# jkulhanek/tetra-nerf

Measured on NVIDIA H100. Metric: rays/sec (4096-ray batch, 300k-tet mesh), higher is better.
Workload: dtype f32 (trace/interp/compositing) + f16w2 tensor-core MLP (fp16 activations x fp16 hi/lo weights, f32 accumulate; per-sample density/colour within 1e-4 of the fp32 oracle, tests/test_gpu_render.py)

## Files before the change

tetra-nerf_b200/csrc/tn_mlp.cuh:

```cuda
#pragma once
#include "tn_common.cuh"
#include "tn_tc.cuh"

namespace tn {

#ifndef TN_MLP_WGS
#define TN_MLP_WGS 3
#endif
constexpr uint32_t MLP_WGS = TN_MLP_WGS;
constexpr uint32_t MLP_THREADS = 128 * MLP_WGS;
constexpr uint32_t MLP_TILE = 64;
constexpr uint32_t MLP_W_BYTES = 32768 + 3 * 65536;
constexpr uint32_t MLP_W_COARSE = 32768 + 2 * 65536;
__host__ __device__ constexpr uint32_t mlp_off_head(bool fine) { return fine ? MLP_W_BYTES : MLP_W_COARSE; }
__host__ __device__ constexpr uint32_t mlp_off_bars(bool fine) { return mlp_off_head(fine) + 520 * 4; }
__host__ __device__ constexpr uint32_t mlp_smem_bytes(bool fine) { return mlp_off_bars(fine) + 8 + 8 * MLP_WGS; }
static_assert(mlp_smem_bytes(true) <= 232448, "k_mlp shared memory exceeds 227 KB");
__host__ __device__ constexpr uint32_t mlp_off_layer(int l) { return l == 0 ? 0u : 32768u + 65536u * (uint32_t)(l - 1); }

struct MlpParams {
    const uint32_t *n_active;
    uint32_t S;
    const uint4 *vi;
    const float *bary;
    const float *fshadow;
    const uint8_t *wimg;
    const float *bias;
    const float *head;
    const float *dirbias;
    float *out;
    uint32_t *tile_ctr;
    const uint32_t *rowmap;
    const uint32_t *n_rows;
};

constexpr uint32_t MLP_NO_TILE = 0xFFFFFFFFu;

__device__ __forceinline__ float softplus_f(float x) { return x > 20.0f ? x : log1pf(expf(x)); }
__device__ __forceinline__ float sigmoid_f(float x) { return 1.0f / (1.0f + expf(-x)); }

__device__ __forceinline__ float4 ldg_stream(const float4 *p) {
    float4 v;
    asm volatile("ld.global.nc.L1::no_allocate.v4.f32 {%0, %1, %2, %3}, [%4];" : "=f"(v.x), "=f"(v.y), "=f"(v.z), "=f"(v.w) : "l"(p));
    return v;
}
__device__ __forceinline__ float4 ldg_l1(const float4 *p) {
    float4 v;
    asm volatile("ld.global.nc.v4.f32 {%0, %1, %2, %3}, [%4];" : "=f"(v.x), "=f"(v.y), "=f"(v.z), "=f"(v.w) : "l"(p));
    return v;
}

template <bool ALLOC_L1>
__device__ __forceinline__ void load_field_quads(const float *__restrict__ row, uint32_t t, float4 (&q)[4]) {
#pragma unroll
    for (int kk = 0; kk < 4; ++kk) {
        const float4 *p = reinterpret_cast<const float4 *>(row + field_pos(16u * kk + 2u * t));
        q[kk] = ALLOC_L1 ? ldg_l1(p) : ldg_stream(p);
    }
}
__device__ __forceinline__ float2 field_pair(const float4 (&q)[4], int c) {
    const float4 v = q[c >> 1];
    return (c & 1) ? make_float2(v.z, v.w) : make_float2(v.x, v.y);
}

__device__ __forceinline__ void wg_sync(uint32_t wg) { asm volatile("bar.sync %0, 128;" ::"r"(1u + wg) : "memory"); }

template <int PREC>
__device__ __forceinline__ void to_operand(float e0, float e1, uint32_t &hi, uint32_t &lo) {
    if (PREC == 2) hi = tc::pack2_f16(e0, e1);
    else tc::split_pack2(e0, e1, hi, lo);
}

struct GatherRows {
    uint4 v[2];
    float b[2][3];
};
__device__ __forceinline__ GatherRows load_gather_rows(const uint4 *__restrict__ vi, const float *__restrict__ bary, uint64_t row0, uint64_t total_rows) {
    GatherRows r;
#pragma unroll
    for (int rr = 0; rr < 2; ++rr) {
        const uint64_t row = row0 + 8u * rr;
        r.v[rr] = make_uint4(TN_EMPTY, TN_EMPTY, TN_EMPTY, TN_EMPTY);
        r.b[rr][0] = r.b[rr][1] = r.b[rr][2] = 0.f;
        if (row < total_rows) {
            r.v[rr] = __ldg(vi + row);
            r.b[rr][0] = __ldg(bary + 3 * row); r.b[rr][1] = __ldg(bary + 3 * row + 1); r.b[rr][2] = __ldg(bary + 3 * row + 2);
        }
    }
    return r;
}
__device__ __forceinline__ GatherRows load_gather_rows_mapped(const uint4 *__restrict__ vi, const float *__restrict__ bary, const uint32_t *__restrict__ rowmap,
                                                          uint64_t row0, uint64_t total_rows) {
    GatherRows r;
#pragma unroll
    for (int rr = 0; rr < 2; ++rr) {
        const uint64_t row = row0 + 8u * rr;
        r.v[rr] = make_uint4(TN_EMPTY, TN_EMPTY, TN_EMPTY, TN_EMPTY);
        r.b[rr][0] = r.b[rr][1] = r.b[rr][2] = 0.f;
        if (row < total_rows) {
            const size_t s = __ldg(rowmap + row);
            r.v[rr] = __ldg(vi + s);
            r.b[rr][0] = __ldg(bary + 3 * s); r.b[rr][1] = __ldg(bary + 3 * s + 1); r.b[rr][2] = __ldg(bary + 3 * s + 2);
        }
    }
    return r;
}
__device__ __forceinline__ void prefetch_l1(const void *p) { asm volatile("prefetch.global.L1 [%0];" ::"l"(p)); }
__device__ __forceinline__ void prefetch_gather_rows(const uint4 *vi, const float *bary, uint64_t row0, uint64_t total_rows) {
#pragma unroll
    for (int rr = 0; rr < 2; ++rr) {
        const uint64_t row = row0 + 8u * rr;
        if (row < total_rows) {
            prefetch_l1(vi + row);
            prefetch_l1(bary + 3 * row);
        }
    }
}

template <int PREC, bool ALLOC_L1 = false>
__device__ __forceinline__ void gather_rows(const GatherRows &r, const float *__restrict__ fshadow, uint32_t t, uint32_t (&xh)[16], uint32_t (&xl)[16]) {
    float4 a[2][4][4];
#pragma unroll
    for (int rr = 0; rr < 2; ++rr) {
        const uint4 v = r.v[rr].x != TN_EMPTY ? r.v[rr] : make_uint4(0u, 0u, 0u, 0u);
        const uint32_t vs[4] = {v.x, v.y, v.z, v.w};
#pragma unroll
        for (int k = 0; k < 4; ++k) load_field_quads<ALLOC_L1>(fshadow + (size_t)vs[k] * 64, t, a[rr][k]);
    }
#pragma unroll
    for (int rr = 0; rr < 2; ++rr) {
        const bool m = r.v[rr].x != TN_EMPTY;
        const float b0 = r.b[rr][0], b1 = r.b[rr][1], b2 = r.b[rr][2];
        const float w0 = __fsub_rn(1.0f, __fadd_rn(__fadd_rn(b0, b1), b2));
#pragma unroll
        for (int c = 0; c < 8; ++c) {
            const float2 a0 = field_pair(a[rr][0], c), a1 = field_pair(a[rr][1], c), a2 = field_pair(a[rr][2], c), a3 = field_pair(a[rr][3], c);
            float2 o;
            o.x = __fmaf_rn(b0, a1.x, 0.f); o.y = __fmaf_rn(b0, a1.y, 0.f);
            o.x = __fmaf_rn(b1, a2.x, o.x); o.y = __fmaf_rn(b1, a2.y, o.y);
            o.x = __fmaf_rn(b2, a3.x, o.x); o.y = __fmaf_rn(b2, a3.y, o.y);
            o.x = __fmaf_rn(w0, a0.x, o.x); o.y = __fmaf_rn(w0, a0.y, o.y);
            if (!m) o = make_float2(0.f, 0.f);
            const int i = 4 * (c >> 1) + 2 * (c & 1) + rr;
            to_operand<PREC>(o.x, o.y, xh[i], xl[i]);
        }
    }
}

template <int PREC, int KSTEPS>
__device__ __forceinline__ void layer_mma(float (&d)[64], const uint32_t (&ah)[4 * KSTEPS], const uint32_t (&al)[4 * KSTEPS], uint32_t w) {
    using namespace tc;
    wgmma_fence();
#pragma unroll
    for (int kk = 0; kk < KSTEPS; ++kk) {
        const uint32_t wb = w + (uint32_t)(kk >> 2) * 32768u + (uint32_t)(kk & 3) * 32u;
        const uint32_t a[4] = {ah[4 * kk], ah[4 * kk + 1], ah[4 * kk + 2], ah[4 * kk + 3]};
        if (PREC == 2) {
            wgmma_rs_f16_n128<0>(d, a, make_desc(wb), kk > 0 ? 1u : 0u);
            wgmma_rs_f16_n128<0>(d, a, make_desc(wb + 16384u), 1u);
        } else {
            const uint32_t b[4] = {al[4 * kk], al[4 * kk + 1], al[4 * kk + 2], al[4 * kk + 3]};
            wgmma_rs_bf16_n128<0>(d, a, make_desc(wb), kk > 0 ? 1u : 0u);
            wgmma_rs_bf16_n128<0>(d, b, make_desc(wb), 1u);
            wgmma_rs_bf16_n128<0>(d, a, make_desc(wb + 16384u), 1u);
        }
    }
    wgmma_commit();
    wgmma_wait0();
    reg_fence(d);
}

template <bool FINE, int PREC, bool MAP = false>
__global__ void __launch_bounds__(MLP_THREADS, 1) k_mlp(const MlpParams p) {
    using namespace tc;
    extern __shared__ __align__(1024) uint8_t tn_mlp_smem[];
    uint8_t *smem = tn_mlp_smem;
    const float *head_s = reinterpret_cast<const float *>(smem + mlp_off_head(FINE));
    uint64_t *w_bar = reinterpret_cast<uint64_t *>(smem + mlp_off_bars(FINE));
    volatile uint32_t *slots = reinterpret_cast<volatile uint32_t *>(smem + mlp_off_bars(FINE) + 8);

    constexpr int L = FINE ? 4 : 3;
    constexpr uint32_t WBYTES = FINE ? MLP_W_BYTES : MLP_W_COARSE;
    const uint32_t wg = threadIdx.x >> 7, tid = threadIdx.x & 127u;
    const uint32_t warp = tid >> 5, lane = threadIdx.x & 31u, g = lane >> 2, t = lane & 3u;
    const uint32_t n_active = *p.n_active;
    const uint64_t total_rows = MAP ? (uint64_t)*p.n_rows : (uint64_t)n_active * p.S;
    const uint32_t ntiles = (uint32_t)((total_rows + MLP_TILE - 1) / MLP_TILE);
    if (blockIdx.x * MLP_WGS >= ntiles) return;
    auto sample_row = [&](uint64_t row) -> uint64_t { return MAP ? (uint64_t)__ldg(p.rowmap + row) : row; };

    if (threadIdx.x == 0) {
        mbar_init(w_bar, 1);
        fence_barrier_init();
    }
    for (uint32_t i = threadIdx.x; i < 516; i += MLP_THREADS) const_cast<float *>(head_s)[i] = p.head[i];
    auto draw = [&]() {
        const uint32_t nx = gridDim.x * MLP_WGS + atomicAdd(p.tile_ctr, 1u);
        return nx < ntiles ? nx : MLP_NO_TILE;
    };
    if (tid == 0) {
        const uint32_t first = blockIdx.x * MLP_WGS + wg;
        slots[2 * wg] = first < ntiles ? first : MLP_NO_TILE;
        slots[2 * wg + 1] = draw();
    }
    __syncthreads();
    if (threadIdx.x == 0) {
        mbar_arrive_expect_tx(w_bar, WBYTES);
        for (uint32_t off = 0; off < WBYTES; off += 16384) tma_bulk_g2s(smem + off, p.wimg + off, 16384, w_bar);
    }
    const uint32_t wsm = smem_u32(smem);
    const float *wd = head_s, *wc = head_s + 128;
    bool weights_ready = false;
    const uint32_t lrow = warp * 16u + g;
    uint32_t tile = slots[2 * wg];

#pragma unroll 1
    for (uint32_t n = 0;; ++n) {
        wg_sync(wg);
        if (tile == MLP_NO_TILE) break;
        const uint32_t next = slots[2 * wg + ((n + 1u) & 1u)];
        if (tid == 0) slots[2 * wg + (n & 1u)] = draw();
        const uint64_t row0 = (uint64_t)tile * MLP_TILE + lrow, row1 = row0 + 8u;
        const float *db0 = nullptr, *db1 = nullptr;

        uint32_t ah[32], al[32];
        {
            uint32_t xh[16], xl[16];
            if constexpr (MAP) gather_rows<PREC, true>(load_gather_rows_mapped(p.vi, p.bary, p.rowmap, row0, total_rows), p.fshadow, t, xh, xl);
            else gather_rows<PREC, true>(load_gather_rows(p.vi, p.bary, row0, total_rows), p.fshadow, t, xh, xl);
            if constexpr (MAP) { if (next != MLP_NO_TILE && lrow == warp * 16u) prefetch_l1(p.rowmap + (uint64_t)next * MLP_TILE + lrow); }
            else if (next != MLP_NO_TILE) prefetch_gather_rows(p.vi, p.bary, (uint64_t)next * MLP_TILE + lrow, total_rows);
            if (FINE) {
                db0 = p.dirbias + (size_t)((uint32_t)sample_row(min(row0, total_rows - 1)) / p.S) * 128;
                db1 = p.dirbias + (size_t)((uint32_t)sample_row(min(row1, total_rows - 1)) / p.S) * 128;
                prefetch_l1(db0 + 32 * t);
                prefetch_l1(db1 + 32 * t);
            }
            if (!weights_ready) { mbar_wait(w_bar, 0); weights_ready = true; }
            float d[64];
            layer_mma<PREC, 4>(d, xh, xl, wsm + mlp_off_layer(0));
#pragma unroll
            for (int j = 0; j < 16; ++j) {
                const float2 b = __ldg(reinterpret_cast<const float2 *>(p.bias + 8 * j + 2 * t));
                const int i = 4 * (j >> 1) + 2 * (j & 1);
                to_operand<PREC>(fmaxf(d[4 * j] + b.x, 0.f), fmaxf(d[4 * j + 1] + b.y, 0.f), ah[i], al[i]);
                to_operand<PREC>(fmaxf(d[4 * j + 2] + b.x, 0.f), fmaxf(d[4 * j + 3] + b.y, 0.f), ah[i + 1], al[i + 1]);
            }
        }
        float dens0 = 0.f, dens1 = 0.f;
#pragma unroll
        for (int l = 1; l < 3; ++l) {
            float d[64];
            layer_mma<PREC, 8>(d, ah, al, wsm + mlp_off_layer(l));
            const float *bias = p.bias + 128 * l;
#pragma unroll
            for (int j = 0; j < 16; ++j) {
                const int c = 8 * j + 2 * (int)t;
                const float2 b = __ldg(reinterpret_cast<const float2 *>(bias + c));
                const float x0 = fmaxf(d[4 * j] + b.x, 0.f), x1 = fmaxf(d[4 * j + 1] + b.y, 0.f);
                const float y0 = fmaxf(d[4 * j + 2] + b.x, 0.f), y1 = fmaxf(d[4 * j + 3] + b.y, 0.f);
                if (l == 2) {
                    dens0 = fmaf(x0, wd[c], dens0); dens0 = fmaf(x1, wd[c + 1], dens0);
                    dens1 = fmaf(y0, wd[c], dens1); dens1 = fmaf(y1, wd[c + 1], dens1);
                }
                if (l < L - 1) {
                    const int i = 4 * (j >> 1) + 2 * (j & 1);
                    to_operand<PREC>(x0, x1, ah[i], al[i]);
                    to_operand<PREC>(y0, y1, ah[i + 1], al[i + 1]);
                }
            }
        }
        float col0[3] = {0.f, 0.f, 0.f}, col1[3] = {0.f, 0.f, 0.f};
        if (FINE) {
            float d[64];
            layer_mma<PREC, 8>(d, ah, al, wsm + mlp_off_layer(3));
#pragma unroll
            for (int j = 0; j < 16; ++j) {
                const int c = 8 * j + 2 * (int)t;
                const float2 b0 = __ldg(reinterpret_cast<const float2 *>(db0 + c)), b1 = __ldg(reinterpret_cast<const float2 *>(db1 + c));
                const float x0 = fmaxf(d[4 * j] + b0.x, 0.f), x1 = fmaxf(d[4 * j + 1] + b0.y, 0.f);
                const float y0 = fmaxf(d[4 * j + 2] + b1.x, 0.f), y1 = fmaxf(d[4 * j + 3] + b1.y, 0.f);
#pragma unroll
                for (int ch = 0; ch < 3; ++ch) {
                    const float *w = wc + 128 * ch;
                    col0[ch] = fmaf(x1, w[c + 1], fmaf(x0, w[c], col0[ch]));
                    col1[ch] = fmaf(y1, w[c + 1], fmaf(y0, w[c], col1[ch]));
                }
            }
        }
#pragma unroll
        for (int s = 1; s <= 2; s <<= 1) {
            dens0 += __shfl_xor_sync(0xffffffffu, dens0, s);
            dens1 += __shfl_xor_sync(0xffffffffu, dens1, s);
            if (FINE) {
#pragma unroll
                for (int ch = 0; ch < 3; ++ch) {
                    col0[ch] += __shfl_xor_sync(0xffffffffu, col0[ch], s);
                    col1[ch] += __shfl_xor_sync(0xffffffffu, col1[ch], s);
                }
            }
        }
        if (t < 2) {
            const uint64_t row = t == 0 ? row0 : row1;
            const float dn = t == 0 ? dens0 : dens1;
            if (row < total_rows) {
                const uint64_t orow = sample_row(row);
                const float sigma = softplus_f(dn + head_s[512]);
                if (FINE) {
                    const float c0 = t == 0 ? col0[0] : col1[0], c1 = t == 0 ? col0[1] : col1[1], c2 = t == 0 ? col0[2] : col1[2];
                    reinterpret_cast<float4 *>(p.out)[orow] =
                        make_float4(sigma, sigmoid_f(c0 + head_s[513]), sigmoid_f(c1 + head_s[514]), sigmoid_f(c2 + head_s[515]));
                } else {
                    p.out[orow] = sigma;
                }
            }
        }
        tile = next;
    }
    if (!weights_ready) mbar_wait(w_bar, 0);
}

template <bool FINE, int PREC, bool MAP = false>
inline int launch_mlp(const MlpParams &p, uint32_t grid, cudaStream_t s) {
    auto k = k_mlp<FINE, PREC, MAP>;
    TN_CUDA(cudaFuncSetAttribute(k, cudaFuncAttributeMaxDynamicSharedMemorySize, (int)mlp_smem_bytes(FINE)));
    k<<<grid, MLP_THREADS, mlp_smem_bytes(FINE), s>>>(p);
    return TN_OK;
}

}
```

tetra-nerf_b200/csrc/tn_tc.cuh:

```cuda
#pragma once
#include <cuda_bf16.h>
#include <cuda_runtime.h>
#include <stdint.h>

namespace tn {
namespace tc {

__device__ __forceinline__ uint32_t smem_u32(const void *p) { return (uint32_t)__cvta_generic_to_shared(p); }

__device__ __forceinline__ void mbar_init(uint64_t *bar, uint32_t count) {
    asm volatile("mbarrier.init.shared::cta.b64 [%0], %1;" ::"r"(smem_u32(bar)), "r"(count));
}
__device__ __forceinline__ void fence_barrier_init() { asm volatile("fence.mbarrier_init.release.cluster;" ::: "memory"); }
__device__ __forceinline__ void mbar_arrive(uint64_t *bar) {
    asm volatile("mbarrier.arrive.shared::cta.b64 _, [%0];" ::"r"(smem_u32(bar)) : "memory");
}
__device__ __forceinline__ void mbar_arrive_expect_tx(uint64_t *bar, uint32_t bytes) {
    asm volatile("mbarrier.arrive.expect_tx.shared::cta.b64 _, [%0], %1;" ::"r"(smem_u32(bar)), "r"(bytes) : "memory");
}
__device__ __forceinline__ bool mbar_test(uint64_t *bar, uint32_t parity) {
    uint32_t ok;
    asm volatile(
        "{\n\t.reg .pred p;\n\t"
        "mbarrier.try_wait.parity.shared::cta.b64 p, [%1], %2;\n\t"
        "selp.u32 %0, 1, 0, p;\n\t}"
        : "=r"(ok)
        : "r"(smem_u32(bar)), "r"(parity)
        : "memory");
    return ok != 0;
}
__device__ __forceinline__ void mbar_wait(uint64_t *bar, uint32_t parity) {
    while (!mbar_test(bar, parity)) {}
}
__device__ __forceinline__ void mbar_wait_backoff(uint64_t *bar, uint32_t parity, uint32_t ns) {
    while (!mbar_test(bar, parity)) __nanosleep(ns);
}

__device__ __forceinline__ bool mbar_test_a(uint32_t bar, uint32_t parity) {
    uint32_t ok;
    asm volatile(
        "{\n\t.reg .pred p;\n\t"
        "mbarrier.try_wait.parity.shared::cta.b64 p, [%1], %2;\n\t"
        "selp.u32 %0, 1, 0, p;\n\t}"
        : "=r"(ok)
        : "r"(bar), "r"(parity)
        : "memory");
    return ok != 0;
}
__device__ __forceinline__ void mbar_wait_a(uint32_t bar, uint32_t parity) {
    while (!mbar_test_a(bar, parity)) {}
}
__device__ __forceinline__ void mbar_wait_backoff_a(uint32_t bar, uint32_t parity, uint32_t ns) {
    while (!mbar_test_a(bar, parity)) __nanosleep(ns);
}

__device__ __forceinline__ void tma_bulk_g2s(void *dst_smem, const void *src_gmem, uint32_t bytes, uint64_t *bar) {
    asm volatile("cp.async.bulk.shared::cluster.global.mbarrier::complete_tx::bytes [%0], [%1], %2, [%3];" ::"r"(smem_u32(dst_smem)),
                 "l"(src_gmem), "r"(bytes), "r"(smem_u32(bar))
                 : "memory");
}

__device__ __forceinline__ void wgmma_fence() { asm volatile("wgmma.fence.sync.aligned;" ::: "memory"); }
__device__ __forceinline__ void wgmma_commit() { asm volatile("wgmma.commit_group.sync.aligned;" ::: "memory"); }
__device__ __forceinline__ void wgmma_wait0() { asm volatile("wgmma.wait_group.sync.aligned 0;" ::: "memory"); }
__device__ __forceinline__ void fence_proxy_async() { asm volatile("fence.proxy.async.shared::cta;" ::: "memory"); }
template <int N>
__device__ __forceinline__ void reg_fence(float (&d)[N]) {
#pragma unroll
    for (int i = 0; i < N; ++i) asm volatile("" : "+f"(d[i])::"memory");
}

__device__ __forceinline__ uint64_t make_desc(uint32_t smem_addr, uint32_t lbo = 16u, uint32_t sbo = 1024u) {
    return (uint64_t)((smem_addr & 0x3FFFFu) >> 4) | ((uint64_t)((lbo >> 4) & 0x3FFFu) << 16) | ((uint64_t)((sbo >> 4) & 0x3FFFu) << 32) |
           (1ull << 62);
}

template <int TB>
__device__ __forceinline__ void wgmma_rs_bf16_n128(float (&d)[64], const uint32_t (&a)[4], uint64_t bdesc, uint32_t acc) {
    asm volatile(
        "{\n\t.reg .pred p;\n\tsetp.ne.b32 p, %69, 0;\n\t"
        "wgmma.mma_async.sync.aligned.m64n128k16.f32.bf16.bf16 "
        "{%0, %1, %2, %3, %4, %5, %6, %7, %8, %9, %10, %11, %12, %13, %14, %15, %16, %17, %18, %19, %20, %21, %22, %23, %24, %25, %26, %27, %28, %29, %30, %31, %32, %33, %34, %35, %36, %37, %38, %39, %40, %41, %42, %43, %44, %45, %46, %47, %48, %49, %50, %51, %52, %53, %54, %55, %56, %57, %58, %59, %60, %61, %62, %63}, "
        "{%64, %65, %66, %67}, %68, p, 1, 1, %70;\n\t}"
        : "+f"(d[0]), "+f"(d[1]), "+f"(d[2]), "+f"(d[3]), "+f"(d[4]), "+f"(d[5]), "+f"(d[6]), "+f"(d[7]), "+f"(d[8]), "+f"(d[9]), "+f"(d[10]), "+f"(d[11]), "+f"(d[12]), "+f"(d[13]), "+f"(d[14]), "+f"(d[15]), "+f"(d[16]), "+f"(d[17]), "+f"(d[18]), "+f"(d[19]), "+f"(d[20]), "+f"(d[21]), "+f"(d[22]), "+f"(d[23]), "+f"(d[24]), "+f"(d[25]), "+f"(d[26]), "+f"(d[27]), "+f"(d[28]), "+f"(d[29]), "+f"(d[30]), "+f"(d[31]), "+f"(d[32]), "+f"(d[33]), "+f"(d[34]), "+f"(d[35]), "+f"(d[36]), "+f"(d[37]), "+f"(d[38]), "+f"(d[39]), "+f"(d[40]), "+f"(d[41]), "+f"(d[42]), "+f"(d[43]), "+f"(d[44]), "+f"(d[45]), "+f"(d[46]), "+f"(d[47]), "+f"(d[48]), "+f"(d[49]), "+f"(d[50]), "+f"(d[51]), "+f"(d[52]), "+f"(d[53]), "+f"(d[54]), "+f"(d[55]), "+f"(d[56]), "+f"(d[57]), "+f"(d[58]), "+f"(d[59]), "+f"(d[60]), "+f"(d[61]), "+f"(d[62]), "+f"(d[63])
        : "r"(a[0]), "r"(a[1]), "r"(a[2]), "r"(a[3]), "l"(bdesc), "r"(acc), "n"(TB));
}
template <int TB>
__device__ __forceinline__ void wgmma_rs_f16_n128(float (&d)[64], const uint32_t (&a)[4], uint64_t bdesc, uint32_t acc) {
    asm volatile(
        "{\n\t.reg .pred p;\n\tsetp.ne.b32 p, %69, 0;\n\t"
        "wgmma.mma_async.sync.aligned.m64n128k16.f32.f16.f16 "
        "{%0, %1, %2, %3, %4, %5, %6, %7, %8, %9, %10, %11, %12, %13, %14, %15, %16, %17, %18, %19, %20, %21, %22, %23, %24, %25, %26, %27, %28, %29, %30, %31, %32, %33, %34, %35, %36, %37, %38, %39, %40, %41, %42, %43, %44, %45, %46, %47, %48, %49, %50, %51, %52, %53, %54, %55, %56, %57, %58, %59, %60, %61, %62, %63}, "
        "{%64, %65, %66, %67}, %68, p, 1, 1, %70;\n\t}"
        : "+f"(d[0]), "+f"(d[1]), "+f"(d[2]), "+f"(d[3]), "+f"(d[4]), "+f"(d[5]), "+f"(d[6]), "+f"(d[7]), "+f"(d[8]), "+f"(d[9]), "+f"(d[10]), "+f"(d[11]), "+f"(d[12]), "+f"(d[13]), "+f"(d[14]), "+f"(d[15]), "+f"(d[16]), "+f"(d[17]), "+f"(d[18]), "+f"(d[19]), "+f"(d[20]), "+f"(d[21]), "+f"(d[22]), "+f"(d[23]), "+f"(d[24]), "+f"(d[25]), "+f"(d[26]), "+f"(d[27]), "+f"(d[28]), "+f"(d[29]), "+f"(d[30]), "+f"(d[31]), "+f"(d[32]), "+f"(d[33]), "+f"(d[34]), "+f"(d[35]), "+f"(d[36]), "+f"(d[37]), "+f"(d[38]), "+f"(d[39]), "+f"(d[40]), "+f"(d[41]), "+f"(d[42]), "+f"(d[43]), "+f"(d[44]), "+f"(d[45]), "+f"(d[46]), "+f"(d[47]), "+f"(d[48]), "+f"(d[49]), "+f"(d[50]), "+f"(d[51]), "+f"(d[52]), "+f"(d[53]), "+f"(d[54]), "+f"(d[55]), "+f"(d[56]), "+f"(d[57]), "+f"(d[58]), "+f"(d[59]), "+f"(d[60]), "+f"(d[61]), "+f"(d[62]), "+f"(d[63])
        : "r"(a[0]), "r"(a[1]), "r"(a[2]), "r"(a[3]), "l"(bdesc), "r"(acc), "n"(TB));
}
template <int TA, int TB>
__device__ __forceinline__ void wgmma_ss_bf16_n128(float (&d)[64], uint64_t adesc, uint64_t bdesc, uint32_t acc) {
    asm volatile(
        "{\n\t.reg .pred p;\n\tsetp.ne.b32 p, %66, 0;\n\t"
        "wgmma.mma_async.sync.aligned.m64n128k16.f32.bf16.bf16 "
        "{%0, %1, %2, %3, %4, %5, %6, %7, %8, %9, %10, %11, %12, %13, %14, %15, %16, %17, %18, %19, %20, %21, %22, %23, %24, %25, %26, %27, %28, %29, %30, %31, %32, %33, %34, %35, %36, %37, %38, %39, %40, %41, %42, %43, %44, %45, %46, %47, %48, %49, %50, %51, %52, %53, %54, %55, %56, %57, %58, %59, %60, %61, %62, %63}, "
        "%64, %65, p, 1, 1, %67, %68;\n\t}"
        : "+f"(d[0]), "+f"(d[1]), "+f"(d[2]), "+f"(d[3]), "+f"(d[4]), "+f"(d[5]), "+f"(d[6]), "+f"(d[7]), "+f"(d[8]), "+f"(d[9]), "+f"(d[10]), "+f"(d[11]), "+f"(d[12]), "+f"(d[13]), "+f"(d[14]), "+f"(d[15]), "+f"(d[16]), "+f"(d[17]), "+f"(d[18]), "+f"(d[19]), "+f"(d[20]), "+f"(d[21]), "+f"(d[22]), "+f"(d[23]), "+f"(d[24]), "+f"(d[25]), "+f"(d[26]), "+f"(d[27]), "+f"(d[28]), "+f"(d[29]), "+f"(d[30]), "+f"(d[31]), "+f"(d[32]), "+f"(d[33]), "+f"(d[34]), "+f"(d[35]), "+f"(d[36]), "+f"(d[37]), "+f"(d[38]), "+f"(d[39]), "+f"(d[40]), "+f"(d[41]), "+f"(d[42]), "+f"(d[43]), "+f"(d[44]), "+f"(d[45]), "+f"(d[46]), "+f"(d[47]), "+f"(d[48]), "+f"(d[49]), "+f"(d[50]), "+f"(d[51]), "+f"(d[52]), "+f"(d[53]), "+f"(d[54]), "+f"(d[55]), "+f"(d[56]), "+f"(d[57]), "+f"(d[58]), "+f"(d[59]), "+f"(d[60]), "+f"(d[61]), "+f"(d[62]), "+f"(d[63])
        : "l"(adesc), "l"(bdesc), "r"(acc), "n"(TA), "n"(TB));
}
template <int TB>
__device__ __forceinline__ void wgmma_rs_bf16_n64(float (&d)[32], const uint32_t (&a)[4], uint64_t bdesc, uint32_t acc) {
    asm volatile(
        "{\n\t.reg .pred p;\n\tsetp.ne.b32 p, %37, 0;\n\t"
        "wgmma.mma_async.sync.aligned.m64n64k16.f32.bf16.bf16 "
        "{%0, %1, %2, %3, %4, %5, %6, %7, %8, %9, %10, %11, %12, %13, %14, %15, %16, %17, %18, %19, %20, %21, %22, %23, %24, %25, %26, %27, %28, %29, %30, %31}, "
        "{%32, %33, %34, %35}, %36, p, 1, 1, %38;\n\t}"
        : "+f"(d[0]), "+f"(d[1]), "+f"(d[2]), "+f"(d[3]), "+f"(d[4]), "+f"(d[5]), "+f"(d[6]), "+f"(d[7]), "+f"(d[8]), "+f"(d[9]), "+f"(d[10]), "+f"(d[11]), "+f"(d[12]), "+f"(d[13]), "+f"(d[14]), "+f"(d[15]), "+f"(d[16]), "+f"(d[17]), "+f"(d[18]), "+f"(d[19]), "+f"(d[20]), "+f"(d[21]), "+f"(d[22]), "+f"(d[23]), "+f"(d[24]), "+f"(d[25]), "+f"(d[26]), "+f"(d[27]), "+f"(d[28]), "+f"(d[29]), "+f"(d[30]), "+f"(d[31])
        : "r"(a[0]), "r"(a[1]), "r"(a[2]), "r"(a[3]), "l"(bdesc), "r"(acc), "n"(TB));
}
template <int TB>
__device__ __forceinline__ void wgmma_rs_f16_n64(float (&d)[32], const uint32_t (&a)[4], uint64_t bdesc, uint32_t acc) {
    asm volatile(
        "{\n\t.reg .pred p;\n\tsetp.ne.b32 p, %37, 0;\n\t"
        "wgmma.mma_async.sync.aligned.m64n64k16.f32.f16.f16 "
        "{%0, %1, %2, %3, %4, %5, %6, %7, %8, %9, %10, %11, %12, %13, %14, %15, %16, %17, %18, %19, %20, %21, %22, %23, %24, %25, %26, %27, %28, %29, %30, %31}, "
        "{%32, %33, %34, %35}, %36, p, 1, 1, %38;\n\t}"
        : "+f"(d[0]), "+f"(d[1]), "+f"(d[2]), "+f"(d[3]), "+f"(d[4]), "+f"(d[5]), "+f"(d[6]), "+f"(d[7]), "+f"(d[8]), "+f"(d[9]), "+f"(d[10]), "+f"(d[11]), "+f"(d[12]), "+f"(d[13]), "+f"(d[14]), "+f"(d[15]), "+f"(d[16]), "+f"(d[17]), "+f"(d[18]), "+f"(d[19]), "+f"(d[20]), "+f"(d[21]), "+f"(d[22]), "+f"(d[23]), "+f"(d[24]), "+f"(d[25]), "+f"(d[26]), "+f"(d[27]), "+f"(d[28]), "+f"(d[29]), "+f"(d[30]), "+f"(d[31])
        : "r"(a[0]), "r"(a[1]), "r"(a[2]), "r"(a[3]), "l"(bdesc), "r"(acc), "n"(TB));
}
template <int TA, int TB>
__device__ __forceinline__ void wgmma_ss_bf16_n64(float (&d)[32], uint64_t adesc, uint64_t bdesc, uint32_t acc) {
    asm volatile(
        "{\n\t.reg .pred p;\n\tsetp.ne.b32 p, %34, 0;\n\t"
        "wgmma.mma_async.sync.aligned.m64n64k16.f32.bf16.bf16 "
        "{%0, %1, %2, %3, %4, %5, %6, %7, %8, %9, %10, %11, %12, %13, %14, %15, %16, %17, %18, %19, %20, %21, %22, %23, %24, %25, %26, %27, %28, %29, %30, %31}, "
        "%32, %33, p, 1, 1, %35, %36;\n\t}"
        : "+f"(d[0]), "+f"(d[1]), "+f"(d[2]), "+f"(d[3]), "+f"(d[4]), "+f"(d[5]), "+f"(d[6]), "+f"(d[7]), "+f"(d[8]), "+f"(d[9]), "+f"(d[10]), "+f"(d[11]), "+f"(d[12]), "+f"(d[13]), "+f"(d[14]), "+f"(d[15]), "+f"(d[16]), "+f"(d[17]), "+f"(d[18]), "+f"(d[19]), "+f"(d[20]), "+f"(d[21]), "+f"(d[22]), "+f"(d[23]), "+f"(d[24]), "+f"(d[25]), "+f"(d[26]), "+f"(d[27]), "+f"(d[28]), "+f"(d[29]), "+f"(d[30]), "+f"(d[31])
        : "l"(adesc), "l"(bdesc), "r"(acc), "n"(TA), "n"(TB));
}

__device__ __forceinline__ void split_pack2(float e0, float e1, uint32_t &hi, uint32_t &lo) {
    uint32_t h, l;
    asm("cvt.rn.bf16x2.f32 %0, %1, %2;" : "=r"(h) : "f"(e1), "f"(e0));
    const float d0 = e0 - __uint_as_float(h << 16), d1 = e1 - __uint_as_float(h & 0xFFFF0000u);
    asm("cvt.rn.bf16x2.f32 %0, %1, %2;" : "=r"(l) : "f"(d1), "f"(d0));
    hi = h;
    lo = l;
}

__device__ __forceinline__ uint32_t pack2_f16(float e0, float e1) {
    uint32_t h;
    asm("cvt.rn.satfinite.f16x2.f32 %0, %1, %2;" : "=r"(h) : "f"(e1), "f"(e0));
    return h;
}

__host__ __device__ inline uint32_t sw128_offset(uint32_t n, uint32_t k) {
    return (n >> 3) * 1024u + (n & 7u) * 128u + ((((k * 2u) >> 4) ^ (n & 7u)) << 4) + ((k * 2u) & 15u);
}

}
}
```

Measured before the change: 4.251 million.

## Split weight TMA into per-layer barriers and fuse ReLU into f16 convert

Weight loading into shared memory now uses one mbarrier per layer, so the first tile can start layer 0 while later layers' weights are still arriving. This hides part of the weight-load latency at kernel start. Separately, ReLU is folded into the f16x2 conversion with cvt.rn.relu.satfinite, which removes the fmaxf instructions. The cost is extra barrier waits on the first tile and a per-layer wait path that is disabled for the FINE PREC==3 variant.

```diff
diff --git a/tetra-nerf_b200/csrc/tn_mlp.cuh b/tetra-nerf_b200/csrc/tn_mlp.cuh
--- a/tetra-nerf_b200/csrc/tn_mlp.cuh
+++ b/tetra-nerf_b200/csrc/tn_mlp.cuh
@@ -14,9 +14,11 @@
 constexpr uint32_t MLP_W_COARSE = 32768 + 2 * 65536;
 __host__ __device__ constexpr uint32_t mlp_off_head(bool fine) { return fine ? MLP_W_BYTES : MLP_W_COARSE; }
 __host__ __device__ constexpr uint32_t mlp_off_bars(bool fine) { return mlp_off_head(fine) + 520 * 4; }
-__host__ __device__ constexpr uint32_t mlp_smem_bytes(bool fine) { return mlp_off_bars(fine) + 8 + 8 * MLP_WGS; }
+__host__ __device__ constexpr uint32_t mlp_off_slots(bool fine) { return mlp_off_bars(fine) + 8 * (fine ? 4 : 3); }
+__host__ __device__ constexpr uint32_t mlp_smem_bytes(bool fine) { return mlp_off_slots(fine) + 8 * MLP_WGS; }
 static_assert(mlp_smem_bytes(true) <= 232448, "k_mlp shared memory exceeds 227 KB");
 __host__ __device__ constexpr uint32_t mlp_off_layer(int l) { return l == 0 ? 0u : 32768u + 65536u * (uint32_t)(l - 1); }
+__host__ __device__ constexpr uint32_t mlp_layer_bytes(int l) { return l == 0 ? 32768u : 65536u; }
 
 struct MlpParams {
     const uint32_t *n_active;
@@ -70,6 +72,11 @@
     if (PREC == 2) hi = tc::pack2_f16(e0, e1);
     else tc::split_pack2(e0, e1, hi, lo);
 }
+template <int PREC>
+__device__ __forceinline__ void to_operand_relu(float e0, float e1, uint32_t &hi, uint32_t &lo) {
+    if (PREC == 2) hi = tc::pack2_f16_relu(e0, e1);
+    else tc::split_pack2(fmaxf(e0, 0.f), fmaxf(e1, 0.f), hi, lo);
+}
 
 struct GatherRows {
     uint4 v[2];
@@ -177,10 +184,10 @@
     uint8_t *smem = tn_mlp_smem;
     const float *head_s = reinterpret_cast<const float *>(smem + mlp_off_head(FINE));
     uint64_t *w_bar = reinterpret_cast<uint64_t *>(smem + mlp_off_bars(FINE));
-    volatile uint32_t *slots = reinterpret_cast<volatile uint32_t *>(smem + mlp_off_bars(FINE) + 8);
+    volatile uint32_t *slots = reinterpret_cast<volatile uint32_t *>(smem + mlp_off_slots(FINE));
 
     constexpr int L = FINE ? 4 : 3;
-    constexpr uint32_t WBYTES = FINE ? MLP_W_BYTES : MLP_W_COARSE;
+    constexpr bool LAYER_WAITS = !(FINE && PREC == 3);
     const uint32_t wg = threadIdx.x >> 7, tid = threadIdx.x & 127u;
     const uint32_t warp = tid >> 5, lane = threadIdx.x & 31u, g = lane >> 2, t = lane & 3u;
     const uint32_t n_active = *p.n_active;
@@ -190,7 +197,7 @@
     auto sample_row = [&](uint64_t row) -> uint64_t { return MAP ? (uint64_t)__ldg(p.rowmap + row) : row; };
 
     if (threadIdx.x == 0) {
-        mbar_init(w_bar, 1);
+        for (int l = 0; l < L; ++l) mbar_init(w_bar + l, 1);
         fence_barrier_init();
     }
     for (uint32_t i = threadIdx.x; i < 516; i += MLP_THREADS) const_cast<float *>(head_s)[i] = p.head[i];
@@ -205,8 +212,11 @@
     }
     __syncthreads();
     if (threadIdx.x == 0) {
-        mbar_arrive_expect_tx(w_bar, WBYTES);
-        for (uint32_t off = 0; off < WBYTES; off += 16384) tma_bulk_g2s(smem + off, p.wimg + off, 16384, w_bar);
+        for (int l = 0; l < L; ++l) {
+            mbar_arrive_expect_tx(w_bar + l, mlp_layer_bytes(l));
+            for (uint32_t off = mlp_off_layer(l); off < mlp_off_layer(l) + mlp_layer_bytes(l); off += 16384)
+                tma_bulk_g2s(smem + off, p.wimg + off, 16384, w_bar + l);
+        }
     }
     const uint32_t wsm = smem_u32(smem);
     const float *wd = head_s, *wc = head_s + 128;
@@ -236,21 +246,25 @@
                 prefetch_l1(db0 + 32 * t);
                 prefetch_l1(db1 + 32 * t);
             }
-            if (!weights_ready) { mbar_wait(w_bar, 0); weights_ready = true; }
+            if (!weights_ready) {
+                if (LAYER_WAITS) mbar_wait(w_bar, 0);
+                else for (int l = 0; l < L; ++l) mbar_wait(w_bar + l, 0);
+            }
             float d[64];
             layer_mma<PREC, 4>(d, xh, xl, wsm + mlp_off_layer(0));
 #pragma unroll
             for (int j = 0; j < 16; ++j) {
                 const float2 b = __ldg(reinterpret_cast<const float2 *>(p.bias + 8 * j + 2 * t));
                 const int i = 4 * (j >> 1) + 2 * (j & 1);
-                to_operand<PREC>(fmaxf(d[4 * j] + b.x, 0.f), fmaxf(d[4 * j + 1] + b.y, 0.f), ah[i], al[i]);
-                to_operand<PREC>(fmaxf(d[4 * j + 2] + b.x, 0.f), fmaxf(d[4 * j + 3] + b.y, 0.f), ah[i + 1], al[i + 1]);
+                to_operand_relu<PREC>(d[4 * j] + b.x, d[4 * j + 1] + b.y, ah[i], al[i]);
+                to_operand_relu<PREC>(d[4 * j + 2] + b.x, d[4 * j + 3] + b.y, ah[i + 1], al[i + 1]);
             }
         }
         float dens0 = 0.f, dens1 = 0.f;
 #pragma unroll
         for (int l = 1; l < 3; ++l) {
             float d[64];
+            if (LAYER_WAITS && !weights_ready) mbar_wait(w_bar + l, 0);
             layer_mma<PREC, 8>(d, ah, al, wsm + mlp_off_layer(l));
             const float *bias = p.bias + 128 * l;
 #pragma unroll
@@ -265,14 +279,20 @@
                 }
                 if (l < L - 1) {
                     const int i = 4 * (j >> 1) + 2 * (j & 1);
-                    to_operand<PREC>(x0, x1, ah[i], al[i]);
-                    to_operand<PREC>(y0, y1, ah[i + 1], al[i + 1]);
+                    if (l == 2) {
+                        to_operand<PREC>(x0, x1, ah[i], al[i]);
+                        to_operand<PREC>(y0, y1, ah[i + 1], al[i + 1]);
+                    } else {
+                        to_operand_relu<PREC>(d[4 * j] + b.x, d[4 * j + 1] + b.y, ah[i], al[i]);
+                        to_operand_relu<PREC>(d[4 * j + 2] + b.x, d[4 * j + 3] + b.y, ah[i + 1], al[i + 1]);
+                    }
                 }
             }
         }
         float col0[3] = {0.f, 0.f, 0.f}, col1[3] = {0.f, 0.f, 0.f};
         if (FINE) {
             float d[64];
+            if (LAYER_WAITS && !weights_ready) mbar_wait(w_bar + 3, 0);
             layer_mma<PREC, 8>(d, ah, al, wsm + mlp_off_layer(3));
 #pragma unroll
             for (int j = 0; j < 16; ++j) {
@@ -315,9 +335,11 @@
                 }
             }
         }
+        weights_ready = true;
         tile = next;
     }
-    if (!weights_ready) mbar_wait(w_bar, 0);
+    if (!weights_ready)
+        for (int l = 0; l < L; ++l) mbar_wait(w_bar + l, 0);
 }
 
 template <bool FINE, int PREC, bool MAP = false>
diff --git a/tetra-nerf_b200/csrc/tn_tc.cuh b/tetra-nerf_b200/csrc/tn_tc.cuh
--- a/tetra-nerf_b200/csrc/tn_tc.cuh
+++ b/tetra-nerf_b200/csrc/tn_tc.cuh
@@ -151,6 +151,12 @@
     return h;
 }
 
+__device__ __forceinline__ uint32_t pack2_f16_relu(float e0, float e1) {
+    uint32_t h;
+    asm("cvt.rn.relu.satfinite.f16x2.f32 %0, %1, %2;" : "=r"(h) : "f"(e1), "f"(e0));
+    return h;
+}
+
 __host__ __device__ inline uint32_t sw128_offset(uint32_t n, uint32_t k) {
     return (n >> 3) * 1024u + (n & 7u) * 128u + ((((k * 2u) >> 4) ^ (n & 7u)) << 4) + ((k * 2u) & 15u);
 }
```

Measured after the change: 4.294 million, median of 6. About the same (+1.0%).
